# chalkydri/chalkydri

Measured on AMD Instinct MI355X. Metric: frames/sec (detect+pose) on 1280x800 batch; HBM GB/s vs roofline, higher is better.
Workload: dtype u8 (threshold/segment/clusters: integer; quad fit/decode/SQPnP: f64)

## Files before the change

### chalkydri_amd/csrc/k_clusters.hip

```cpp
#include "ck_internal.h"

namespace {

constexpr int NT = 256;
constexpr int ETW = 64, ETH = 16;
constexpr int LW = ETW + 2, LH = ETH + 1;
constexpr int LHT = 512;
constexpr uint32_t SKIP = 0xFFFFFFFFu;

__device__ __forceinline__ uint32_t key_hash(unsigned long long k) {
    uint32_t x = (uint32_t)((k >> 32) ^ k);
    x *= 2654435761u;
    return x ^ (x >> 15);
}

struct EmitArgs {
    const uint8_t *thresh;
    const ck_label_t *labels;
    const uint32_t *groot, *gsize;
    size_t slots;
    int w, h, tiles_x, tiles_y, min_comp;
    int ccl_tiles_x;
    int stop_after;
    ck_stage_ws ws;
};

__device__ __forceinline__ void lds_barrier() { asm volatile("s_waitcnt lgkmcnt(0)\n\ts_barrier" ::: "memory"); }

__global__ __launch_bounds__(NT) void k_emit(EmitArgs a) {
    __shared__ uint8_t sT[LH][LW + 2];
    __shared__ uint32_t sR[LH][LW];
    __shared__ unsigned long long sKey[LHT];
    __shared__ uint32_t sCnt[LHT], sSlot[LHT], sTBase[LHT];
    __shared__ uint32_t sWave[NT / 64 + 1], sRunW[NT / 64 + 1];
    const int tid = threadIdx.x;
    const int tiles = a.tiles_x * a.tiles_y;
    const int frame = blockIdx.x / tiles, tile = blockIdx.x - frame * tiles;
    const int ty = tile / a.tiles_x, tx = tile - ty * a.tiles_x;
    const int x0 = tx * ETW, y0 = ty * ETH;
    const int w = a.w, h = a.h;
    const size_t npix = (size_t)w * h;
    const uint8_t *T = a.thresh + (size_t)frame * npix;
    const ck_label_t *L = a.labels + (size_t)frame * npix;
    const uint32_t *GR = a.groot + (size_t)frame * a.slots, *GS = a.gsize + (size_t)frame * a.slots;
    const ck_stage_ws &ws = a.ws;
    unsigned long long *gkeys = ws.d_ht_keys + (size_t)frame * ws.ht_size;
    uint32_t *gcount = ws.d_ht_count + (size_t)frame * ws.ht_size;
    uint32_t *counters = ws.d_counters + (size_t)frame * CK_CNT_STRIDE;
    ck_packed_point *tmp = ws.d_tmp + (size_t)frame * ws.ext_cap;
    ck_run *runs = ws.d_runs + (size_t)frame * ws.run_cap;

    for (int i = tid; i < LHT; i += NT) { sKey[i] = 0ull; sCnt[i] = 0; }
    {
        constexpr int SPT = (LH * LW + NT - 1) / NT;
        uint32_t lab[SPT], hop[SPT], csz[SPT], slot[SPT];
        uint8_t tv[SPT];
#pragma unroll
        for (int q = 0; q < SPT; q++) {
            const int i = tid + q * NT;
            const int ly = i / LW, lx = i - ly * LW;
            const int gy = y0 + ly, gx = x0 - 1 + lx;
            tv[q] = 127; lab[q] = CK_LBL_NONE; slot[q] = 0;
            if (i < LH * LW && gy < h && gx >= 0 && gx < w) {
                const uint32_t p = (uint32_t)gy * (uint32_t)w + (uint32_t)gx;
                tv[q] = T[p]; lab[q] = L[p];
                slot[q] = ck_label_slot(lab[q], gx, gy, a.ccl_tiles_x);
            }
        }
#pragma unroll
        for (int q = 0; q < SPT; q++) {
            const bool two = tv[q] != 127 && !(lab[q] & CK_LBL_SMALL) && (lab[q] & CK_LBL_BORDER);
            hop[q] = two ? GR[slot[q]] : CK_LBL_INVALID;
            csz[q] = two ? GS[slot[q]] : 0u;
        }
#pragma unroll
        for (int q = 0; q < SPT; q++) {
            const int i = tid + q * NT;
            if (i >= LH * LW) continue;
            const int ly = i / LW, lx = i - ly * LW;
            uint32_t r = SKIP;
            if (tv[q] != 127 && !(lab[q] & CK_LBL_SMALL)) {
                if (lab[q] & CK_LBL_BORDER) r = ((int)csz[q] < a.min_comp) ? SKIP : hop[q];
                else r = ck_label_interior_root(lab[q], x0 - 1 + lx, y0 + ly, w);
            }
            sT[ly][lx] = tv[q];
            sR[ly][lx] = r;
        }
    }
    lds_barrier();
    if (a.stop_after == 0) return;

    const int lx = (tid & 63) + 1;
    const int gx = x0 + (tid & 63);
    const int row0 = (tid >> 6) * 4;
    const int dxs[4] = {1, 0, -1, 1}, dys[4] = {0, 1, 1, 1};
    const bool colok = gx >= 1 && gx <= w - 2;

    constexpr uint32_t NONE = 0xFFFFFFFFu;
    uint32_t cand[16];
#pragma unroll
    for (int q = 0; q < 16; q++) cand[q] = NONE;
    if (colok) {
#pragma unroll
        for (int rr = 0; rr < 4; rr++) {
            int ly = row0 + rr, gy = y0 + ly;
            if (gy < 1 || gy > h - 2) continue;
            int v0 = sT[ly][lx];
            uint32_t r0 = sR[ly][lx];
            if (r0 == SKIP) continue;
            uint32_t r1v[4];
            bool ok[4];
#pragma unroll
            for (int k = 0; k < 4; k++) {
                const int v1 = sT[ly + dys[k]][lx + dxs[k]];
                r1v[k] = sR[ly + dys[k]][lx + dxs[k]];
                ok[k] = (v0 + v1 == 255) && r1v[k] != SKIP;
            }
#pragma unroll
            for (int k = 0; k < 4; k++) {
                bool leader = ok[k];
#pragma unroll
                for (int j = 0; j < k; j++) leader = leader && !(ok[j] && r1v[j] == r1v[k]);
                if (!leader) continue;
                uint32_t n = 1;
#pragma unroll
                for (int j = k + 1; j < 4; j++) n += (ok[j] && r1v[j] == r1v[k]) ? 1u : 0u;
                const uint32_t r1 = r1v[k];
                unsigned long long key = r0 < r1 ? ((unsigned long long)r0 << 32) | r1 : ((unsigned long long)r1 << 32) | r0;
                uint32_t s = key_hash(key) & (LHT - 1);
                bool placed = false;
                for (int probe = 0; probe < LHT; probe++) {
                    __asm__ volatile("" ::: "memory");
                    unsigned long long prev = sKey[s];
                    if (prev == 0ull) prev = atomicCAS(&sKey[s], 0ull, key);
                    if (prev == 0ull || prev == key) {
                        uint32_t c = (s << 16) | atomicAdd(&sCnt[s], n);
                        cand[rr * 4 + k] = c;
#pragma unroll
                        for (int j = k + 1; j < 4; j++)
                            if (ok[j] && r1v[j] == r1) cand[rr * 4 + j] = ++c;
                        placed = true;
                        break;
                    }
                    s = (s + 1) & (LHT - 1);
                }
                if (!placed) atomicOr(&counters[CK_CNT_STATUS], (uint32_t)CK_FRAME_CLUSTERS_OVERFLOW);
            }
        }
    }
    lds_barrier();
    if (a.stop_after == 1) return;

    const unsigned long long k0 = sKey[2 * tid], k1 = sKey[2 * tid + 1];
    const uint32_t c0 = k0 ? sCnt[2 * tid] : 0u, c1 = k1 ? sCnt[2 * tid + 1] : 0u;
    uint32_t found0 = SKIP, found1 = SKIP, ridx0;
    {
        const uint32_t incl = wave_scan_u32(c0 + c1);
        const unsigned long long b0 = __ballot(k0 != 0ull), b1 = __ballot(k1 != 0ull);
        const unsigned long long below = (1ull << (tid & 63)) - 1ull;
        ridx0 = (uint32_t)(__popcll(b0 & below) + __popcll(b1 & below));
        if ((tid & 63) == 63) sWave[tid >> 6] = incl;
        if ((tid & 63) == 0) sRunW[tid >> 6] = (uint32_t)(__popcll(b0) + __popcll(b1));
        lds_barrier();
        uint32_t before = 0, total = 0, rbefore = 0, rtotal = 0;
#pragma unroll
        for (int wv = 0; wv < NT / 64; wv++) {
            uint32_t t = sWave[wv], r = sRunW[wv];
            if (wv < (tid >> 6)) { before += t; rbefore += r; }
            total += t; rtotal += r;
        }
        ridx0 += rbefore;
        lds_barrier();
        if (tid == 0) {
            sWave[NT / 64] = total ? atomicAdd(&counters[CK_CNT_TMP], total) : 0u;
            sRunW[NT / 64] = rtotal ? atomicAdd(&counters[CK_CNT_RUNS], rtotal) : 0u;
        }
        const uint32_t excl = before + incl - (c0 + c1);
        sTBase[2 * tid] = excl; sTBase[2 * tid + 1] = excl + c0;
        {
            const uint32_t hm = (uint32_t)(ws.ht_size - 1);
            const uint32_t g0 = key_hash(k0) & hm, g1 = key_hash(k1) & hm;
            const unsigned long long p0 = k0 ? atomicCAS(&gkeys[g0], 0ull, k0) : 0ull;
            const unsigned long long p1 = k1 ? atomicCAS(&gkeys[g1], 0ull, k1) : 0ull;
#pragma unroll
            for (int q = 0; q < 2; q++) {
                const unsigned long long key = q ? k1 : k0, pv = q ? p1 : p0;
                if (key == 0ull) continue;
                uint32_t g = q ? g1 : g0, found = SKIP;
                if (pv == 0ull || pv == key) found = g;
                else {
                    for (int probe = 1; probe < ws.ht_size; probe++) {
                        g = (g + 1) & hm;
                        unsigned long long prev = atomicCAS(&gkeys[g], 0ull, key);
                        if (prev == 0ull || prev == key) { found = g; break; }
                    }
                }
                if (found == SKIP) atomicOr(&counters[CK_CNT_STATUS], (uint32_t)CK_FRAME_CLUSTERS_OVERFLOW);
                sSlot[2 * tid + q] = found;
                if (q) found1 = found; else found0 = found;
            }
        }
        if (found0 != SKIP) atomicAdd(&gcount[found0], c0);
        if (found1 != SKIP) atomicAdd(&gcount[found1], c1);
    }
    lds_barrier();
    if (a.stop_after == 2) return;

    const uint32_t tile_base = sWave[NT / 64];
    if (colok) {
#pragma unroll
        for (int rr = 0; rr < 4; rr++) {
            int ly = row0 + rr, gy = y0 + ly;
#pragma unroll
            for (int k = 0; k < 4; k++) {
                const uint32_t cd = cand[rr * 4 + k];
                if (cd == NONE) continue;
                const uint32_t s = cd >> 16, lr = cd & 0xFFFFu;
                uint32_t slot = sSlot[s];
                if (slot == SKIP) continue;
                uint32_t ti = tile_base + sTBase[s] + lr;
                if (ti >= (uint32_t)ws.point_cap) { atomicOr(&counters[CK_CNT_STATUS], (uint32_t)CK_FRAME_POINTS_OVERFLOW); continue; }
                int v0 = sT[ly][lx], v1 = sT[ly + dys[k]][lx + dxs[k]];
                tmp[ti] = ((uint32_t)(2 * gx + dxs[k]) << 16) | ((uint32_t)(2 * gy + dys[k]) << 3) | ((uint32_t)k << 1) | (v1 > v0 ? 1u : 0u);
            }
        }
    }
    {
        uint32_t ri = sRunW[NT / 64] + ridx0;
#pragma unroll
        for (int q = 0; q < 2; q++) {
            if ((q ? k1 : k0) == 0ull) continue;
            const uint32_t found = q ? found1 : found0;
            if (ri < (uint32_t)ws.run_cap) {
                ck_run r;
                r.slot = found != SKIP ? found : 0u; r.base = 0; r.tmp_start = tile_base + sTBase[2 * tid + q];
                r.count = found != SKIP ? (q ? c1 : c0) : 0u;
                runs[ri] = r;
            } else if (found != SKIP) atomicOr(&counters[CK_CNT_STATUS], (uint32_t)CK_FRAME_CLUSTERS_OVERFLOW);
            ri++;
        }
    }
}

constexpr uint32_t ID_WHITE = 0x40000000u, ID_VALUE = 0x3FFFFFFFu;
constexpr int SR_PAD = ((LH * LW + NT - 1) / NT) * NT;

__global__ __launch_bounds__(NT) __attribute__((amdgpu_num_sgpr(80))) void k_emit2(EmitArgs a, int xcd_map, int n_frames) {
    __shared__ __attribute__((aligned(16))) uint32_t sRaw[SR_PAD + LHT * 2 + LHT];
    __shared__ uint32_t sSlot[LHT], sTBase[LHT];
    __shared__ uint32_t sWave[NT / 64 + 1], sRunW[NT / 64 + 1];
    uint32_t *sR = sRaw;
    unsigned long long *sKey = reinterpret_cast<unsigned long long *>(sRaw + SR_PAD);
    uint32_t *sCnt = sRaw + SR_PAD + LHT * 2;
    const int tid = threadIdx.x;
    const int tiles = a.tiles_x * a.tiles_y;
    int frame, tile;
    if (xcd_map) {
        const int x = blockIdx.x & 7, j = blockIdx.x >> 3;
        frame = (j / tiles) * 8 + x; tile = j % tiles;
        if (frame >= n_frames) return;
    } else { frame = blockIdx.x / tiles; tile = blockIdx.x - frame * tiles; }
    const int ty = tile / a.tiles_x, tx = tile - ty * a.tiles_x;
    const int x0 = tx * ETW, y0 = ty * ETH;
    const int w = a.w, h = a.h;
    const size_t npix = (size_t)w * h;
    const uint8_t *T = a.thresh + (size_t)frame * npix;
    const ck_label_t *L = a.labels + (size_t)frame * npix;
    const uint32_t *GR = a.groot + (size_t)frame * a.slots, *GS = a.gsize + (size_t)frame * a.slots;
    const ck_stage_ws &ws = a.ws;
    unsigned long long *gkeys = ws.d_ht_keys + (size_t)frame * ws.ht_size;
    uint32_t *gcount = ws.d_ht_count + (size_t)frame * ws.ht_size;
    uint32_t *counters = ws.d_counters + (size_t)frame * CK_CNT_STRIDE;
    ck_packed_point *tmp = ws.d_tmp + (size_t)frame * ws.ext_cap;
    ck_run *runs = ws.d_runs + (size_t)frame * ws.run_cap;

    for (int i = tid; i < LHT; i += NT) { sKey[i] = 0ull; sCnt[i] = 0; }
    {
        constexpr int SPT = SR_PAD / NT;
        uint32_t lab[SPT], tv[SPT], slot[SPT], hop[SPT], csz[SPT];
        bool inb[SPT];
        int gxs[SPT], gys[SPT];
#pragma unroll
        for (int q = 0; q < SPT; q++) {
            const int i = tid + q * NT;
            const int ly = i / LW, lx = i - ly * LW;
            const int gy = y0 + ly, gx = x0 - 1 + lx;
            inb[q] = i < LH * LW && gy < h && gx >= 0 && gx < w;
            const int cy = min(gy, h - 1), cx = min(max(gx, 0), w - 1);
            const uint32_t p = (uint32_t)cy * (uint32_t)w + (uint32_t)cx;
            tv[q] = T[p]; lab[q] = L[p];
            gxs[q] = cx; gys[q] = cy;
        }
#pragma unroll
        for (int q = 0; q < SPT; q++) {
            const bool two = inb[q] && tv[q] != 127u && !(lab[q] & CK_LBL_SMALL) && (lab[q] & CK_LBL_BORDER);
            slot[q] = two ? ck_label_slot(lab[q], gxs[q], gys[q], a.ccl_tiles_x) : 0u;
            hop[q] = GR[slot[q]]; csz[q] = GS[slot[q]];
        }
#pragma unroll
        for (int q = 0; q < SPT; q++) {
            const bool brd = (lab[q] & CK_LBL_BORDER) != 0u;
            const bool none = !inb[q] || tv[q] == 127u || (lab[q] & CK_LBL_SMALL) || (brd && (int)csz[q] < a.min_comp);
            const uint32_t root = brd ? hop[q] : ck_label_interior_root(lab[q], gxs[q], gys[q], w);
            sR[tid + q * NT] = none ? SKIP : (root | (tv[q] == 255u ? ID_WHITE : 0u));
        }
    }
    lds_barrier();
    if (a.stop_after == 0) return;

    const int lx = (tid & 63) + 1;
    const int gx = x0 + (tid & 63);
    const int row0 = (tid >> 6) * 4;
    const bool colok = gx >= 1 && gx <= w - 2;

    constexpr uint32_t NONE = 0xFFFFFFFFu;
    uint32_t cand[16];
    {
        uint32_t R[5][3];
        unsigned long long last_key = 0ull;
        uint32_t last_s = 0;
#pragma unroll
        for (int r = 0; r < 5; r++)
#pragma unroll
            for (int c = 0; c < 3; c++) R[r][c] = sR[(row0 + r) * LW + lx - 1 + c];
#pragma unroll
        for (int rr = 0; rr < 4; rr++) {
            const int gy = y0 + row0 + rr;
            const uint32_t r0 = (colok && gy >= 1 && gy <= h - 2) ? R[rr][1] : SKIP;
            const uint32_t r1v[4] = {R[rr][2], R[rr + 1][1], R[rr + 1][0], R[rr + 1][2]};
            bool ok[4];
#pragma unroll
            for (int k = 0; k < 4; k++) ok[k] = r0 != SKIP && r1v[k] != SKIP && ((r0 ^ r1v[k]) & ID_WHITE) != 0u;
            uint32_t lead[4], nth[4], mult[4];
#pragma unroll
            for (int k = 0; k < 4; k++) {
                lead[k] = (uint32_t)k; nth[k] = 0; mult[k] = 1;
#pragma unroll
                for (int j = k - 1; j >= 0; j--) { const bool eq = ok[j] && r1v[j] == r1v[k]; lead[k] = eq ? (uint32_t)j : lead[k]; nth[k] += eq ? 1u : 0u; }
#pragma unroll
                for (int j = k + 1; j < 4; j++) mult[k] += (ok[j] && r1v[j] == r1v[k]) ? 1u : 0u;
            }
            uint32_t cl[4] = {NONE, NONE, NONE, NONE};
#pragma unroll
            for (int k = 0; k < 4; k++) {
                if (!(ok[k] && lead[k] == (uint32_t)k)) continue;
                const uint32_t ra = r0 & ID_VALUE, rb = r1v[k] & ID_VALUE;
                const unsigned long long key = ra < rb ? ((unsigned long long)ra << 32) | rb : ((unsigned long long)rb << 32) | ra;
                uint32_t s = key_hash(key) & (LHT - 1);
                bool placed = false;
                if (key == last_key) { placed = true; s = last_s; }
                else
                for (int probe = 0; probe < LHT; probe++) {
                    __asm__ volatile("" ::: "memory");
                    unsigned long long prev = sKey[s];
                    if (prev == 0ull) prev = atomicCAS(&sKey[s], 0ull, key);
                    if (prev == 0ull || prev == key) { placed = true; break; }
                    s = (s + 1) & (LHT - 1);
                }
                if (placed) { last_key = key; last_s = s; }
                if (placed) cl[k] = (s << 16) | atomicAdd(&sCnt[s], mult[k]);
                else atomicOr(&counters[CK_CNT_STATUS], (uint32_t)CK_FRAME_CLUSTERS_OVERFLOW);
            }
#pragma unroll
            for (int k = 0; k < 4; k++) {
                const uint32_t lk = lead[k];
                const uint32_t c = lk == 0u ? cl[0] : (lk == 1u ? cl[1] : (lk == 2u ? cl[2] : cl[3]));
                const uint32_t sign = (r1v[k] & ID_WHITE) ? 0x80000000u : 0u;
                cand[rr * 4 + k] = (ok[k] && c != NONE) ? ((c + nth[k]) | sign) : NONE;
            }
        }
    }
    lds_barrier();
    if (a.stop_after == 1) return;

    const unsigned long long k0 = sKey[2 * tid], k1 = sKey[2 * tid + 1];
    const uint32_t c0 = k0 ? sCnt[2 * tid] : 0u, c1 = k1 ? sCnt[2 * tid + 1] : 0u;
    uint32_t found0 = SKIP, found1 = SKIP, ridx0, tile_total;
    {
        const uint32_t incl = wave_scan_u32(c0 + c1);
        const unsigned long long b0 = __ballot(k0 != 0ull), b1 = __ballot(k1 != 0ull);
        const unsigned long long below = (1ull << (tid & 63)) - 1ull;
        ridx0 = (uint32_t)(__popcll(b0 & below) + __popcll(b1 & below));
        if ((tid & 63) == 63) sWave[tid >> 6] = incl;
        if ((tid & 63) == 0) sRunW[tid >> 6] = (uint32_t)(__popcll(b0) + __popcll(b1));
        lds_barrier();
        uint32_t before = 0, total = 0, rbefore = 0, rtotal = 0;
#pragma unroll
        for (int wv = 0; wv < NT / 64; wv++) {
            uint32_t t = sWave[wv], r = sRunW[wv];
            if (wv < (tid >> 6)) { before += t; rbefore += r; }
            total += t; rtotal += r;
        }
        ridx0 += rbefore;
        tile_total = total;
        if (tid == 0) {
            sWave[NT / 64] = total ? atomicAdd(&counters[CK_CNT_TMP], total) : 0u;
            sRunW[NT / 64] = rtotal ? atomicAdd(&counters[CK_CNT_RUNS], rtotal) : 0u;
        }
        const uint32_t excl = before + incl - (c0 + c1);
        sTBase[2 * tid] = excl; sTBase[2 * tid + 1] = excl + c0;
        {
            const uint32_t hm = (uint32_t)(ws.ht_size - 1);
            const uint32_t g0 = key_hash(k0) & hm, g1 = key_hash(k1) & hm;
            const unsigned long long p0 = k0 ? atomicCAS(&gkeys[g0], 0ull, k0) : 0ull;
            const unsigned long long p1 = k1 ? atomicCAS(&gkeys[g1], 0ull, k1) : 0ull;
#pragma unroll
            for (int q = 0; q < 2; q++) {
                const unsigned long long key = q ? k1 : k0, pv = q ? p1 : p0;
                uint32_t found = SKIP;
                if (key != 0ull) {
                    uint32_t g = q ? g1 : g0;
                    if (pv == 0ull || pv == key) found = g;
                    else {
                        for (int probe = 1; probe < ws.ht_size; probe++) {
                            g = (g + 1) & hm;
                            unsigned long long prev = atomicCAS(&gkeys[g], 0ull, key);
                            if (prev == 0ull || prev == key) { found = g; break; }
                        }
                    }
                    if (found == SKIP) atomicOr(&counters[CK_CNT_STATUS], (uint32_t)CK_FRAME_CLUSTERS_OVERFLOW);
                }
                sSlot[2 * tid + q] = found;
                if (q) found1 = found; else found0 = found;
            }
        }
        if (found0 != SKIP) atomicAdd(&gcount[found0], c0);
        if (found1 != SKIP) atomicAdd(&gcount[found1], c1);
    }
    lds_barrier();
    if (a.stop_after == 2) return;

    const uint32_t tile_base = sWave[NT / 64];
    (void)tile_total;
#pragma unroll
    for (int q = 0; q < 16; q++) {
        const uint32_t cd = cand[q];
        if (cd == NONE) continue;
        const int rr = q >> 2, k = q & 3;
        const int dxk = k == 1 ? 0 : (k == 2 ? -1 : 1), dyk = k == 0 ? 0 : 1;
        const uint32_t s = (cd >> 16) & 0x3FFu, lr = cd & 0xFFFFu;
        if (sSlot[s] == SKIP) continue;
        const uint32_t ti = tile_base + sTBase[s] + lr;
        if (ti >= (uint32_t)ws.point_cap) { atomicOr(&counters[CK_CNT_STATUS], (uint32_t)CK_FRAME_POINTS_OVERFLOW); continue; }
        const int gy = y0 + row0 + rr;
        tmp[ti] = ((uint32_t)(2 * gx + dxk) << 16) | ((uint32_t)(2 * gy + dyk) << 3) | ((uint32_t)k << 1) | (cd >> 31);
    }
    {
        uint32_t ri = sRunW[NT / 64] + ridx0;
#pragma unroll
        for (int q = 0; q < 2; q++) {
            if ((q ? k1 : k0) == 0ull) continue;
            const uint32_t found = q ? found1 : found0;
            if (ri < (uint32_t)ws.run_cap) {
                ck_run r;
                r.slot = found != SKIP ? found : 0u; r.base = 0; r.tmp_start = tile_base + (q ? sTBase[2 * tid + 1] : sTBase[2 * tid]);
                r.count = found != SKIP ? (q ? c1 : c0) : 0u;
                runs[ri] = r;
            } else if (found != SKIP) atomicOr(&counters[CK_CNT_STATUS], (uint32_t)CK_FRAME_CLUSTERS_OVERFLOW);
            ri++;
        }
    }
}

__global__ __launch_bounds__(NT) void k_clear(uint4 *keys4, size_t nkeys4, uint4 *cnt4, size_t ncnt4, uint32_t *c0, uint32_t n0, uint32_t *c1,
                                              uint32_t n1, uint32_t *c2, uint32_t n2) {
    const size_t i = (size_t)blockIdx.x * NT + threadIdx.x;
    const uint4 z = make_uint4(0, 0, 0, 0);
    if (i < nkeys4) keys4[i] = z;
    else if (i - nkeys4 < ncnt4) cnt4[i - nkeys4] = z;
    if (i < n0) c0[i] = 0;
    if (i < n1) c1[i] = 0;
    if (i < n2) c2[i] = 0;
}

constexpr int SNT = 1024;
__global__ __launch_bounds__(SNT) void k_scan(ck_stage_ws ws, int min_cluster, int max_cluster) {
    __shared__ uint32_t sPts[SNT / 64], sCl[SNT / 64];
    const int frame = blockIdx.x, tid = threadIdx.x, lane = tid & 63, wv = tid >> 6;
    const unsigned long long *gkeys = ws.d_ht_keys + (size_t)frame * ws.ht_size;
    const uint32_t *gcount = ws.d_ht_count + (size_t)frame * ws.ht_size;
    uint32_t *goff = ws.d_ht_off + (size_t)frame * ws.ht_size;
    uint32_t *counters = ws.d_counters + (size_t)frame * CK_CNT_STRIDE;
    ck_cluster_t *clusters = ws.d_clusters + (size_t)frame * ws.cluster_cap;
    const int seg = ws.ht_size / (SNT / 64);
    const int base = wv * seg;
    uint32_t pts = 0, cl = 0;
#pragma unroll 8
    for (int r = 0; r < seg; r += 64) {
        uint32_t c = gcount[base + r + lane];
        bool ok = (int)c >= min_cluster && (int)c <= max_cluster;
        pts += ok ? c : 0u; cl += ok ? 1u : 0u;
    }
    pts = (uint32_t)__builtin_amdgcn_readlane((int)wave_scan_u32(pts), 63);
    cl = (uint32_t)__builtin_amdgcn_readlane((int)wave_scan_u32(cl), 63);
    if (lane == 0) { sPts[wv] = pts; sCl[wv] = cl; }
    __syncthreads();
    uint32_t po = 0, co = 0;
    for (int k = 0; k < wv; k++) { po += sPts[k]; co += sCl[k]; }
    for (int r4 = 0; r4 < seg; r4 += 256) {
        uint32_t c4[4];
#pragma unroll
        for (int q = 0; q < 4; q++) c4[q] = r4 + 64 * q < seg ? gcount[base + r4 + 64 * q + lane] : 0u;
#pragma unroll
    for (int q = 0; q < 4; q++) {
        const int r = r4 + 64 * q;
        if (r >= seg) continue;
        const int e = base + r + lane;
        const uint32_t c = c4[q];
        const bool ok = (int)c >= min_cluster && (int)c <= max_cluster;
        const uint32_t ip = wave_scan_u32(ok ? c : 0u), ic = wave_scan_u32(ok ? 1u : 0u);
        uint32_t off = SKIP;
        if (ok) {
            const uint32_t my_po = po + ip - c, my_co = co + ic - 1u;
            if (my_co < (uint32_t)ws.cluster_cap && my_po + c <= (uint32_t)ws.point_cap) {
                off = my_po;
                unsigned long long key = gkeys[e];
                ck_cluster_t ck;
                ck.rep0 = (uint32_t)(key >> 32); ck.rep1 = (uint32_t)key; ck.start = my_po; ck.count = c;
                clusters[my_co] = ck;
            } else {
                if (my_co < (uint32_t)ws.cluster_cap) {
                    ck_cluster_t ck;
                    ck.rep0 = 0; ck.rep1 = 0; ck.start = 0; ck.count = 0;
                    clusters[my_co] = ck;
                }
                atomicOr(&counters[CK_CNT_STATUS], (uint32_t)CK_FRAME_CLUSTERS_OVERFLOW);
            }
        }
        goff[e] = off;
        po += (uint32_t)__builtin_amdgcn_readlane((int)ip, 63);
        co += (uint32_t)__builtin_amdgcn_readlane((int)ic, 63);
    }
    }
    if (tid == SNT - 1) {
        counters[CK_CNT_CLUSTERS] = min(co, (uint32_t)ws.cluster_cap);
        counters[CK_CNT_POINTS] = min(po, (uint32_t)ws.point_cap);
    }
}

template <int RPW>
__global__ __launch_bounds__(NT) void k_scatter(ck_stage_ws ws) {
    const int frame = blockIdx.y;
    const uint32_t *counters = ws.d_counters + (size_t)frame * CK_CNT_STRIDE;
    const uint32_t nruns = min(counters[CK_CNT_RUNS], (uint32_t)ws.run_cap);
    const uint32_t ntmp = min(counters[CK_CNT_TMP], (uint32_t)ws.point_cap);
    const ck_packed_point *tmp = ws.d_tmp + (size_t)frame * ws.ext_cap;
    const ck_run *runs = ws.d_runs + (size_t)frame * ws.run_cap;
    uint32_t *goff = ws.d_ht_off + (size_t)frame * ws.ht_size;
    ck_packed_point *pts = ws.d_points + (size_t)frame * ws.ext_cap;
    const int lane = threadIdx.x & 63;
    const uint32_t wave = blockIdx.x * (NT / 64) + (threadIdx.x >> 6), nwaves = gridDim.x * (NT / 64);
    for (uint32_t r0 = wave * RPW; r0 < nruns; r0 += nwaves * RPW) {
        ck_run mine = {0, 0, 0, 0};
        uint32_t moff = SKIP;
        if (lane < RPW && r0 + lane < nruns) { mine = runs[r0 + lane]; moff = goff[mine.slot]; }
        if (moff == SKIP) mine.count = 0;
        const uint32_t dst0 = mine.count ? atomicAdd(&goff[mine.slot], mine.count) : 0u;
        const unsigned long long small = __ballot(mine.count > 0 && mine.count <= 64);
        unsigned long long todo = small;
        const int sub = lane >> 4, sl = lane & 15;
        while (todo) {
            unsigned long long t = todo;
            int pick = -1;
#pragma unroll
            for (int q = 0; q < 4; q++) {
                const int bit = t ? __builtin_ctzll(t) : -1;
                if (q == sub) pick = bit;
                if (t) t &= t - 1;
            }
            todo = t;
            const int srcl = pick < 0 ? 0 : pick;
            const uint32_t cnt = (uint32_t)__shfl((int)mine.count, srcl, 64), ts = (uint32_t)__shfl((int)mine.tmp_start, srcl, 64),
                           ds = (uint32_t)__shfl((int)dst0, srcl, 64);
            ck_packed_point v[4];
            bool ok[4];
#pragma unroll
            for (int q = 0; q < 4; q++) {
                const uint32_t j = (uint32_t)sl + 16u * q;
                ok[q] = pick >= 0 && j < cnt && ts + j < ntmp;
                v[q] = ok[q] ? tmp[ts + j] : 0u;
            }
#pragma unroll
            for (int q = 0; q < 4; q++)
                if (ok[q]) pts[ds + (uint32_t)sl + 16u * q] = v[q];
        }
        unsigned long long big = __ballot(mine.count > 64);
        while (big) {
            const int srcl = __builtin_ctzll(big);
            big &= big - 1;
            const uint32_t cnt = (uint32_t)__builtin_amdgcn_readlane((int)mine.count, srcl), ts = (uint32_t)__builtin_amdgcn_readlane((int)mine.tmp_start, srcl),
                           ds = (uint32_t)__builtin_amdgcn_readlane((int)dst0, srcl);
            for (uint32_t j0 = 0; j0 < cnt; j0 += 256) {
                ck_packed_point v[4];
                bool ok[4];
#pragma unroll
                for (int q = 0; q < 4; q++) {
                    const uint32_t j = j0 + (uint32_t)lane + 64u * q;
                    ok[q] = j < cnt && ts + j < ntmp;
                    v[q] = ok[q] ? tmp[ts + j] : 0u;
                }
#pragma unroll
                for (int q = 0; q < 4; q++)
                    if (ok[q]) pts[ds + j0 + (uint32_t)lane + 64u * q] = v[q];
            }
        }
    }
}

}

int ck_launch_clusters(ck_handle *h, int n) {
    ck_stage_ws &ws = h->ws;
    {
        const ck_fit_layout fl = ck_fit_scratch_layout(ws, h->cfg.max_batch);
        const size_t nkeys4 = (size_t)ws.ht_size * n / 2, ncnt4 = (size_t)ws.ht_size * n / 4;
        const size_t total4 = nkeys4 + ncnt4;
        hipLaunchKernelGGL(k_clear, dim3((unsigned)((total4 + NT - 1) / NT)), dim3(NT), 0, h->stream,
                           reinterpret_cast<uint4 *>(ws.d_ht_keys), nkeys4, reinterpret_cast<uint4 *>(ws.d_ht_count), ncnt4, ws.d_counters,
                           (uint32_t)(CK_CNT_STRIDE * n), fl.list_counts, 32u, fl.cand_count, (uint32_t)n);
    }
    EmitArgs a;
    a.thresh = h->d_thresh; a.labels = h->d_labels; a.groot = h->d_groot; a.gsize = h->d_gsize; a.slots = (size_t)h->broot_cap;
    a.w = h->qw; a.h = h->qh; a.tiles_x = (h->qw + ETW - 1) / ETW; a.tiles_y = (h->qh + ETH - 1) / ETH;
    a.min_comp = h->cfg.min_component_px; a.ws = ws; a.ccl_tiles_x = h->tiles_x;
    { static const int stop_after = CK_KNOB("CK_EMIT_STOP_AFTER", 99); a.stop_after = stop_after; }
    static const int emit_v = CK_KNOB("CK_EMIT_V", 2);
    static const int emit_xcd = CK_KNOB("CK_EMIT_XCD", -1);
    if (emit_v == 1) hipLaunchKernelGGL(k_emit, dim3((unsigned)(a.tiles_x * a.tiles_y * n)), dim3(NT), 0, h->stream, a);
    else {
        const int xcd_map = emit_xcd >= 0 ? emit_xcd : (n >= 16 ? 1 : 0);
        const unsigned grid = xcd_map ? (unsigned)(((n + 7) / 8) * 8 * a.tiles_x * a.tiles_y) : (unsigned)(a.tiles_x * a.tiles_y * n);
        hipLaunchKernelGGL(k_emit2, dim3(grid), dim3(NT), 0, h->stream, a, xcd_map, n);
    }
    int min_cluster = h->cfg.min_cluster_pixels < 24 ? 24 : h->cfg.min_cluster_pixels;
    hipLaunchKernelGGL(k_scan, dim3((unsigned)n), dim3(SNT), 0, h->stream, ws, min_cluster, ws.max_cluster_points);
    if (n <= 4) hipLaunchKernelGGL(k_scatter<8>, dim3(256u, (unsigned)n), dim3(NT), 0, h->stream, ws);
    else {
        static const unsigned sc_wgs = (unsigned)CK_KNOB("CK_SCATTER_WGS", 32);
        hipLaunchKernelGGL(k_scatter<64>, dim3(sc_wgs, (unsigned)n), dim3(NT), 0, h->stream, ws);
    }
    CK_HIP(hipGetLastError());
    return CK_OK;
}
```

Before: 18610.

## Stage emit tile with vectorized four-pixel loads and padded LDS rows

Interior emit tiles in k_emit2 now load four threshold bytes and four labels per thread with a single 32-bit and a single 64-bit load, replacing per-pixel gathers. Root and slot bases are computed once per tile because an emit tile lies inside one segmentation tile. The halo row and columns are handled by an extra group of threads. The LDS staging row is padded to 72 words so the main body can be written with uint4 stores, and block-index divisions now use precomputed magic-number fastdiv. This adds a second code path plus alignment and bounds gating, so edge tiles still take the old path.

```diff
diff --git a/chalkydri_amd/csrc/k_clusters.hip b/chalkydri_amd/csrc/k_clusters.hip
--- a/chalkydri_amd/csrc/k_clusters.hip
+++ b/chalkydri_amd/csrc/k_clusters.hip
@@ -13,6 +13,14 @@
     x *= 2654435761u;
     return x ^ (x >> 15);
 }
+
+struct FastDiv { uint32_t m, s; };
+inline FastDiv fastdiv_of(uint32_t d) {
+    uint32_t l = 0;
+    while ((1u << l) < d) l++;
+    return {(uint32_t)(((1ull << (31 + l)) + d - 1) / d), 31 + l};
+}
+__device__ __forceinline__ uint32_t fastdiv(uint32_t n, FastDiv f) { return (uint32_t)(((unsigned long long)n * f.m) >> f.s); }
 
 struct EmitArgs {
     const uint8_t *thresh;
@@ -21,6 +29,7 @@
     size_t slots;
     int w, h, tiles_x, tiles_y, min_comp;
     int ccl_tiles_x;
+    FastDiv div_tiles, div_tiles_x;
     int stop_after;
     ck_stage_ws ws;
 };
@@ -243,24 +252,40 @@
 }
 
 constexpr uint32_t ID_WHITE = 0x40000000u, ID_VALUE = 0x3FFFFFFFu;
-constexpr int SR_PAD = ((LH * LW + NT - 1) / NT) * NT;
+constexpr int LP = 72, LB = 4;
+constexpr int SR_WORDS = LH * LP;
+static_assert(ETW == 64 && ETH == 16 && NT == ETH * (ETW / 4), "staging by groups of four: thread t = row t >> 4, group t & 15");
+static_assert(CK_TW % ETW == 0 && CK_TH % ETH == 0, "an emit tile lies inside one segmentation tile");
+static_assert(ETW + 2 * LH <= 2 * 64 && SR_WORDS % 2 == 0, "the row below and the halo columns fit two waves; the keys stay 8-byte aligned");
+
+__device__ __forceinline__ uint32_t staged_id(uint32_t tv, uint32_t lab, bool inb, uint32_t hop, uint32_t csz, uint32_t interior_root, int min_comp) {
+    const bool brd = (lab & CK_LBL_BORDER) != 0u;
+    const bool none = !inb || tv == 127u || (lab & CK_LBL_SMALL) || (brd && (int)csz < min_comp);
+    return none ? SKIP : ((brd ? hop : interior_root) | (tv == 255u ? ID_WHITE : 0u));
+}
+__device__ __forceinline__ uint32_t staged_id_in(uint32_t white, uint32_t lab, bool two, uint32_t hop, uint32_t csz, uint32_t interior_root, uint32_t gate) {
+    const uint32_t x = two ? csz : ((lab >> 14) & 1u) - 1u;
+    const uint32_t id = (two ? hop : interior_root) | white;
+    return x < gate ? SKIP : id;
+}
 
 __global__ __launch_bounds__(NT) __attribute__((amdgpu_num_sgpr(80))) void k_emit2(EmitArgs a, int xcd_map, int n_frames) {
-    __shared__ __attribute__((aligned(16))) uint32_t sRaw[SR_PAD + LHT * 2 + LHT];
+    __shared__ __attribute__((aligned(16))) uint32_t sRaw[SR_WORDS + LHT * 2 + LHT];
     __shared__ uint32_t sSlot[LHT], sTBase[LHT];
     __shared__ uint32_t sWave[NT / 64 + 1], sRunW[NT / 64 + 1];
     uint32_t *sR = sRaw;
-    unsigned long long *sKey = reinterpret_cast<unsigned long long *>(sRaw + SR_PAD);
-    uint32_t *sCnt = sRaw + SR_PAD + LHT * 2;
+    unsigned long long *sKey = reinterpret_cast<unsigned long long *>(sRaw + SR_WORDS);
+    uint32_t *sCnt = sRaw + SR_WORDS + LHT * 2;
     const int tid = threadIdx.x;
     const int tiles = a.tiles_x * a.tiles_y;
     int frame, tile;
     if (xcd_map) {
         const int x = blockIdx.x & 7, j = blockIdx.x >> 3;
-        frame = (j / tiles) * 8 + x; tile = j % tiles;
+        const int q = (int)fastdiv((uint32_t)j, a.div_tiles);
+        frame = q * 8 + x; tile = j - q * tiles;
         if (frame >= n_frames) return;
-    } else { frame = blockIdx.x / tiles; tile = blockIdx.x - frame * tiles; }
-    const int ty = tile / a.tiles_x, tx = tile - ty * a.tiles_x;
+    } else { frame = (int)fastdiv(blockIdx.x, a.div_tiles); tile = blockIdx.x - frame * tiles; }
+    const int ty = (int)fastdiv((uint32_t)tile, a.div_tiles_x), tx = tile - ty * a.tiles_x;
     const int x0 = tx * ETW, y0 = ty * ETH;
     const int w = a.w, h = a.h;
     const size_t npix = (size_t)w * h;
@@ -275,9 +300,58 @@
     ck_run *runs = ws.d_runs + (size_t)frame * ws.run_cap;
 
     for (int i = tid; i < LHT; i += NT) { sKey[i] = 0ull; sCnt[i] = 0; }
-    {
-        constexpr int SPT = SR_PAD / NT;
-        uint32_t lab[SPT], tv[SPT], slot[SPT], hop[SPT], csz[SPT];
+    const bool by_fours = x0 + ETW <= w && y0 + ETH <= h && (w & 3) == 0 &&
+                          ((reinterpret_cast<uintptr_t>(T) & 3u) | (reinterpret_cast<uintptr_t>(L) & 7u)) == 0u;
+    if (by_fours) {
+        const bool extra = tid < 2 * 64;
+        const int hp = tid - ETW;
+        const int r = tid >> 4, g = tid & 15;
+        const uint32_t p = (uint32_t)(y0 + r) * (uint32_t)w + (uint32_t)(x0 + 4 * g);
+        const uint32_t t4 = *reinterpret_cast<const uint32_t *>(T + p);
+        const uint2 l4 = *reinterpret_cast<const uint2 *>(L + p);
+        uint32_t tvx = 0u, labx = CK_LBL_NONE, hopx = 0u, cszx = 0u, slotx = 0u, rootx = 0u;
+        if (extra) {
+            const int gy = y0 + (hp < 0 ? ETH : hp >> 1), gx = hp < 0 ? x0 + tid : ((hp & 1) ? x0 + ETW : x0 - 1);
+            const bool inbx = hp < 2 * LH && gy < h && gx >= 0 && gx < w;
+            const uint32_t cy = (uint32_t)min(gy, h - 1), cx = (uint32_t)min(max(gx, 0), w - 1);
+            const uint32_t px = cy * (uint32_t)w + cx;
+            tvx = T[px];
+            labx = inbx ? (uint32_t)L[px] : CK_LBL_NONE;
+            slotx = ((cy / CK_TH) * (uint32_t)a.ccl_tiles_x + cx / CK_TW) * (uint32_t)CK_RING_CAP;
+            rootx = (cy & ~(uint32_t)(CK_TH - 1)) * (uint32_t)w + (cx & ~(uint32_t)(CK_TW - 1));
+        }
+        const uint32_t slot0 = (uint32_t)((y0 / CK_TH) * a.ccl_tiles_x + x0 / CK_TW) * (uint32_t)CK_RING_CAP;
+        const uint32_t root0 = (uint32_t)(y0 & ~(CK_TH - 1)) * (uint32_t)w + (uint32_t)(x0 & ~(CK_TW - 1));
+        const uint32_t gate = (uint32_t)max(a.min_comp, 1);
+        uint32_t lab[4], hop[4], csz[4], id[4];
+        bool two[4];
+#pragma unroll
+        for (int k = 0; k < 4; k++) lab[k] = ((k & 2 ? l4.y : l4.x) >> (16 * (k & 1))) & 0xFFFFu;
+#pragma unroll
+        for (int k = 0; k < 4; k++) {
+            two[k] = (lab[k] & (CK_LBL_SMALL | CK_LBL_BORDER)) == CK_LBL_BORDER;
+            const uint32_t off = two[k] ? (slot0 + (lab[k] & CK_LBL_ID_MASK)) * 4u : 0u;
+            hop[k] = *reinterpret_cast<const uint32_t *>(reinterpret_cast<const char *>(GR) + off);
+            csz[k] = *reinterpret_cast<const uint32_t *>(reinterpret_cast<const char *>(GS) + off);
+        }
+        const bool twox = (labx & (CK_LBL_SMALL | CK_LBL_BORDER)) == CK_LBL_BORDER;
+        if (extra) {
+            const uint32_t off = twox ? (slotx + (labx & CK_LBL_ID_MASK)) * 4u : 0u;
+            hopx = *reinterpret_cast<const uint32_t *>(reinterpret_cast<const char *>(GR) + off);
+            cszx = *reinterpret_cast<const uint32_t *>(reinterpret_cast<const char *>(GS) + off);
+        }
+#pragma unroll
+        for (int k = 0; k < 4; k++) {
+            const uint32_t white = (k < 3 ? t4 << (23 - 8 * k) : t4 >> 1) & ID_WHITE;
+            id[k] = staged_id_in(white, lab[k], two[k], hop[k], csz[k], root0 + ((lab[k] >> 7) & (CK_TH - 1)) * (uint32_t)w + (lab[k] & (CK_TW - 1)), gate);
+        }
+        *reinterpret_cast<uint4 *>(&sR[r * LP + LB + 4 * g]) = make_uint4(id[0], id[1], id[2], id[3]);
+        if (extra && hp < 2 * LH)
+            sR[hp < 0 ? ETH * LP + LB + tid : (hp >> 1) * LP + ((hp & 1) ? LB + ETW : LB - 1)] =
+                staged_id_in((tvx << 23) & ID_WHITE, labx, twox, hopx, cszx, rootx + ((labx >> 7) & (CK_TH - 1)) * (uint32_t)w + (labx & (CK_TW - 1)), gate);
+    } else {
+        constexpr int SPT = (LH * LW + NT - 1) / NT;
+        uint32_t lab[SPT], tv[SPT], hop[SPT], csz[SPT];
         bool inb[SPT];
         int gxs[SPT], gys[SPT];
 #pragma unroll
@@ -294,15 +368,15 @@
 #pragma unroll
         for (int q = 0; q < SPT; q++) {
             const bool two = inb[q] && tv[q] != 127u && !(lab[q] & CK_LBL_SMALL) && (lab[q] & CK_LBL_BORDER);
-            slot[q] = two ? ck_label_slot(lab[q], gxs[q], gys[q], a.ccl_tiles_x) : 0u;
-            hop[q] = GR[slot[q]]; csz[q] = GS[slot[q]];
+            const uint32_t slot = two ? ck_label_slot(lab[q], gxs[q], gys[q], a.ccl_tiles_x) : 0u;
+            hop[q] = GR[slot]; csz[q] = GS[slot];
         }
 #pragma unroll
         for (int q = 0; q < SPT; q++) {
-            const bool brd = (lab[q] & CK_LBL_BORDER) != 0u;
-            const bool none = !inb[q] || tv[q] == 127u || (lab[q] & CK_LBL_SMALL) || (brd && (int)csz[q] < a.min_comp);
-            const uint32_t root = brd ? hop[q] : ck_label_interior_root(lab[q], gxs[q], gys[q], w);
-            sR[tid + q * NT] = none ? SKIP : (root | (tv[q] == 255u ? ID_WHITE : 0u));
+            const int i = tid + q * NT;
+            const int ly = i / LW, lx = i - ly * LW;
+            const uint32_t id = staged_id(tv[q], lab[q], inb[q], hop[q], csz[q], ck_label_interior_root(lab[q], gxs[q], gys[q], w), a.min_comp);
+            if (i < LH * LW) sR[ly * LP + LB - 1 + lx] = id;
         }
     }
     lds_barrier();
@@ -322,7 +396,7 @@
 #pragma unroll
         for (int r = 0; r < 5; r++)
 #pragma unroll
-            for (int c = 0; c < 3; c++) R[r][c] = sR[(row0 + r) * LW + lx - 1 + c];
+            for (int c = 0; c < 3; c++) R[r][c] = sR[(row0 + r) * LP + LB - 1 + lx - 1 + c];
 #pragma unroll
         for (int rr = 0; rr < 4; rr++) {
             const int gy = y0 + row0 + rr;
@@ -623,6 +697,7 @@
     a.thresh = h->d_thresh; a.labels = h->d_labels; a.groot = h->d_groot; a.gsize = h->d_gsize; a.slots = (size_t)h->broot_cap;
     a.w = h->qw; a.h = h->qh; a.tiles_x = (h->qw + ETW - 1) / ETW; a.tiles_y = (h->qh + ETH - 1) / ETH;
     a.min_comp = h->cfg.min_component_px; a.ws = ws; a.ccl_tiles_x = h->tiles_x;
+    a.div_tiles = fastdiv_of((uint32_t)(a.tiles_x * a.tiles_y)); a.div_tiles_x = fastdiv_of((uint32_t)a.tiles_x);
     { static const int stop_after = CK_KNOB("CK_EMIT_STOP_AFTER", 99); a.stop_after = stop_after; }
     static const int emit_v = CK_KNOB("CK_EMIT_V", 2);
     static const int emit_xcd = CK_KNOB("CK_EMIT_XCD", -1);
```

Result: no change. 18760 (median of 6 runs) (+0.8%).
